# multiplefish/VPLines-SLAM

Hardware: AMD Instinct MI355X
Metric: sliding-window BA solves/sec (10 KF, 200 pts + 80 lines, 5 iters) (higher is better)
Workload: dtype f64

## Files before the change

vplines-slam_amd/csrc/ba_stage.h:

```cpp
#pragma once
#include <hip/hip_runtime.h>

#include <algorithm>
#include <cstring>
#include <memory>
#include <vector>

struct CopySeg {
  const char* src;
  char* dst;
  unsigned bytes;
  unsigned u0;
};
static_assert(sizeof(CopySeg) == 24, "CopySeg layout");

__global__ __launch_bounds__(256) void k_copy_segments(const CopySeg* tab, int nseg, unsigned total_units) {
  for (unsigned u = blockIdx.x * 256u + threadIdx.x; u < total_units; u += gridDim.x * 256u) {
    int lo = 0, hi = nseg - 1;
    while (lo < hi) {
      const int mid = (lo + hi + 1) >> 1;
      if (tab[mid].u0 <= u) lo = mid; else hi = mid - 1;
    }
    const CopySeg sg = tab[lo];
    const unsigned off = (u - sg.u0) * 16u;
    const unsigned rem = sg.bytes - off;
    const char* src = sg.src + off;
    char* dst = sg.dst + off;
    if (rem >= 16u && (((uintptr_t)src | (uintptr_t)dst) & 15u) == 0) {
      *reinterpret_cast<uint4*>(dst) = *reinterpret_cast<const uint4*>(src);
    } else {
      const unsigned nb = rem < 16u ? rem : 16u;
      for (unsigned b = 0; b < nb; b += 4) *reinterpret_cast<uint32_t*>(dst + b) = *reinterpret_cast<const uint32_t*>(src + b);
    }
  }
}

template <typename T>
struct Span {
  T* p = nullptr;
  size_t n = 0;
  T& operator[](size_t i) const { return p[i]; }
  T* data() const { return p; }
  size_t size() const { return n; }
  bool empty() const { return n == 0; }
  T* begin() const { return p; }
  T* end() const { return p + n; }
};

struct Stage {
  char* h = nullptr;
  char* d = nullptr;
  size_t cap = 0, used = 0;
  std::vector<CopySeg> segs;
  unsigned units = 0;
  bool overflow = false;
  bool dry = false;
  std::vector<std::unique_ptr<char[]>> spill;

  hipError_t reserve(size_t need) {
    used = 0; segs.clear(); units = 0; overflow = false; spill.clear();
    if (need <= cap) return hipSuccess;
    release();
    const size_t want = need + need / 4 + (1u << 16);
    hipError_t e = hipHostMalloc((void**)&h, want, hipHostMallocDefault);
    if (e != hipSuccess) return e;
    e = hipMalloc((void**)&d, want);
    if (e != hipSuccess) return e;
    cap = want;
    return hipSuccess;
  }
  void release() {
    if (h) (void)hipHostFree(h);
    if (d) (void)hipFree(d);
    h = d = nullptr; cap = 0;
  }
  size_t bound() const { return ((used + 63) & ~(size_t)63) + segs.size() * sizeof(CopySeg); }
  template <typename T>
  Span<T> take(size_t n) {
    used = (used + 63) & ~(size_t)63;
    Span<T> sp;
    sp.n = n;
    if (!dry && used + n * sizeof(T) <= cap) sp.p = reinterpret_cast<T*>(h + used);
    else if (!dry) { overflow = true; spill.emplace_back(new char[n * sizeof(T) + 1]); sp.p = reinterpret_cast<T*>(spill.back().get()); }
    used += n * sizeof(T);
    return sp;
  }
  template <typename T>
// ... 52 lines not shown
```

vplines-slam_amd/csrc/ba_step.h:

```cpp
#pragma once
#include "ba_common.h"
#include "ba_solve.h"

namespace vpl {

constexpr int SCHUR_THREADS = 256;
constexpr int CHOL_THREADS = 256;
constexpr int BACK_THREADS = 256;

__device__ __forceinline__ void lds_ticket_wait(int* t, int seq) {
  while (__hip_atomic_load(t, __ATOMIC_RELAXED, __HIP_MEMORY_SCOPE_WORKGROUP) != seq) __builtin_amdgcn_s_sleep(1);
  __builtin_amdgcn_fence(__ATOMIC_ACQUIRE, "workgroup", "local");
}
__device__ __forceinline__ void lds_ticket_pass(int* t, int seq, int lane) {
  __builtin_amdgcn_fence(__ATOMIC_RELEASE, "workgroup", "local");
  if (lane == 0) __hip_atomic_store(t, seq + 1, __ATOMIC_RELAXED, __HIP_MEMORY_SCOPE_WORKGROUP);
}

__device__ __forceinline__ int compact2vis(int c, int s, int WS) {
  if (c < WS - 6) { const int v = 6 * s + c; return v < 66 ? v : -1; }
  if (c < WS) return 66 + (c - (WS - 6));
  return c < WS + 2 ? 72 + (c - WS) : -1;
}

// ... 542 lines not shown
__global__ __launch_bounds__(SCHUR_THREADS, 2) void k_schur_mixed(DevBatch B) {
  extern __shared__ double sm[];
  if (blockIdx.x == 0 && threadIdx.x == 0) { B.ord_cnt[2 * ((B.ord_it + 1) & 1)] = 0; B.ord_cnt[2 * ((B.ord_it + 1) & 1) + 1] = 0; }
  schur_body<3, true>(B, ordered_window(B), sm);
}
inline size_t schur_smem(int maxP, int maxL, int ntc = 5) {
  const int r1 = std::max(4 * maxP + 28 * maxL, (int)CSQ_N);
  const int maxKS = maxP / 4 + maxL + NF + 2;
  return (size_t)(r1 + 3 * maxP + 22 * maxL + 176 + 24) * sizeof(double) + (size_t)(8 + 4 * maxKS + ntc * (ntc + 1) / 2 * 256) * sizeof(int);
}

constexpr int DN = 90;
constexpr int DNT = 6;
constexpr int DNAP = DNT * (DNT + 1) / 2 * 256;
constexpr int XLD = 80;
constexpr int CHOL_MIN_WAVES = 2;
constexpr int XROWS_A = 36, XROWS_B = 48;
__device__ __forceinline__ constexpr int xcol(int ch, int J) { return ch == 0 ? 16 * (J > 3 ? J - 1 : J) : 16 * (J - 1); }
__device__ __forceinline__ constexpr int tile_row(int t) { return t < 1 ? 0 : t < 3 ? 1 : t < 6 ? 2 : t < 10 ? 3 : t < 15 ? 4 : 5; }

__device__ __forceinline__ int chain_frame(int ch, int b) { return ch == 0 ? 1 + b : 10 - b; }
__device__ __forceinline__ int chain_col(int ch, int b, int lane) {
  if (lane < 18) {
    const int ds = (b & 1) ? 9 : 0;
    const int f = chain_frame(ch, b);
    const int fr = (lane >= ds && lane < ds + 9) ? f : (ch == 0 ? f + 1 : f - 1);
    return 15 * fr + 6 + (lane < 9 ? lane : lane - 9);
  }
  if (ch == 0) {
    if (lane < 27) return 6 + (lane - 18);
    if (lane < 63) return 15 * ((lane - 27) / 6) + (lane - 27) % 6;
    return NC;
  }
  if (lane < 54) return 15 * (5 + (lane - 18) / 6) + (lane - 18) % 6;
  return lane == 54 ? NC : -1;
}
__device__ __forceinline__ int cam2dense(int c) {
  if (c < 0) return -1;
  if (c == NC) return DN;
  const int v = cam2vis(c);
  if (v >= 0) return v;
  if (c < 15) return 72 + (c - 6);
  return (c >= 81 && c < 90) ? c : -1;
}
__device__ __forceinline__ int dense2cam(int d) { return d < NV ? vis2cam(d) : (d < 81 ? 6 + (d - 72) : d); }
__device__ __forceinline__ int chain_dense(int ch, int lane) {
  if (lane < 18) {
    const bool s5 = ch == 0 ? lane < 9 : lane >= 9;
    return s5 ? 81 + (lane < 9 ? lane : lane - 9) : -1;
  }
  return cam2dense(chain_col(ch, 0, lane));
}

__device__ __forceinline__ void chol_body(const DevBatch& B, const int w, double* sm) {
  const int tid = threadIdx.x, T = CHOL_THREADS;
  const int lane = tid & 63, wv = ((tid >> 6) + ((blockIdx.x >> 8) & 1) * 2) & 3;
  TrState* tr = &B.tr[w];
  if (tr->status != 0 || tr->reuse != 0 || B.path[w] != 0) return;
  count_active(B, 1);
  constexpr int REG = (XROWS_A + XROWS_B) * XLD > DNAP ? (XROWS_A + XROWS_B) * XLD : DNAP;
  double* XA = sm;
  double* XBm = sm + XROWS_A * XLD;
  double* S = sm;
  double* scv = sm + REG;
  double* dgv = scv + 176;
  double* ycam = dgv + 176;
  double* yv = ycam + 176;
  double* isd = yv + 96;
  double* Linv = isd + 96;
  double* red = Linv + 256;
  int* flag = (int*)(red + 24);
  double* rsL = (double*)(flag + 8);

  const size_t fb = (size_t)w * B.nfull;
  const double* gscale = B.scale + fb;
  const double* gdiag = B.diag + fb;
  const double* ggrad = B.grad + fb;
  double* ggn = B.gn + fb;
  const double* Hcc = B.Hcc + (size_t)w * NCP;
  const double* gc = B.gc + (size_t)w * NC;
  const double* sacc = B.sacc + (size_t)w * SACC_N;
  const double mu = tr->mu;
  for (int c = tid; c < 176; c += T) { scv[c] = c < NC ? gscale[c] : 0.0; dgv[c] = c < NC ? gdiag[c] : 1.0; ycam[c] = 0.0; }
  if (tid < 4) flag[tid] = 0;
  for (int i = tid; i < (XROWS_A + XROWS_B) * XLD; i += T) sm[i] = 0.0;
  __syncthreads();
  VPL_STAMP(B, w, 8);

  double U[45];
#pragma unroll
  for (int i = 0; i < 45; ++i) U[i] = 0.0;
#define Xs(b, k) U[9 * (b) + (k)]
  if (wv < 2) {
    const int ch = wv, nblk = ch == 0 ? 4 : 5;
    double* Xout = ch == 0 ? XA : XBm;
    const int xd = chain_dense(ch, lane);
    const int xp = xd < 0 ? -1 : xcol(ch, xd >> 4) + (xd & 15);
    bool bad = false;
    auto load_strip = [&](int b, double (&raw)[9]) {
      const int col = chain_col(ch, b, lane);
      const int f = chain_frame(ch, b);
#pragma unroll
      for (int i = 0; i < 9; ++i) {
        const int r = 15 * f + 6 + i;
        raw[i] = 0.0;
        if (col == NC) raw[i] = gc[r];
        else if (col >= 0) raw[i] = Hcc[col > r ? tri(col, r) : tri(r, col)];
      }
    };
    double rawn[9];
    load_strip(0, rawn);
#pragma unroll
    for (int b = 0; b < 5; ++b) {
      if (b < nblk) {
        const int ds = (b & 1) ? 9 : 0, ns = 9 - ds;
        const int col = chain_col(ch, b, lane);
        const int f = chain_frame(ch, b);
        double R[9];
        {
          const double scol = col == NC ? 1.0 : (col >= 0 ? scv[col] : 0.0);
#pragma unroll
          for (int i = 0; i < 9; ++i) {
            const int r = 15 * f + 6 + i;
            R[i] = rawn[i] * (scv[r] * scol);
            if (col == r) R[i] += mu * dgv[r] * dgv[r];
          }
        }
        if (b + 1 < nblk) load_strip(b + 1, rawn);
        if (b > 0) {
          const bool fresh = lane >= ns && lane < ns + 9;
#pragma unroll
          for (int k = 0; k < 9; ++k) {
            const double xk = fresh ? 0.0 : Xs(b - 1, k);
#pragma unroll
            for (int i = 0; i < 9; ++i) R[i] -= readlane_f64(Xs(b - 1, k), ds + i) * xk;
          }
        }
// ... 77 lines not shown
#pragma unroll 1
    for (int ks = 0; ks < XROWS_B / 4; ++ks) {
      const int need = min(5, (4 * ks + 3) / 9 + 1);
      while (have < need) {
        have = __hip_atomic_load(&flag[2], __ATOMIC_RELAXED, __HIP_MEMORY_SCOPE_WORKGROUP);
        if (have >= need) __builtin_amdgcn_fence(__ATOMIC_ACQUIRE, "workgroup");
      }
      const double* row = XBm + (4 * ks + kk) * XLD + m;
      double x[6];
#pragma unroll
      for (int J = 0; J < 6; ++J) x[J] = J == 0 ? 0.0 : row[xcol(1, J)];
#pragma unroll
      for (int t = 0; t < 21; ++t) {
        const int I = tile_row(t), J = t - I * (I + 1) / 2;
        if ((t & 1) != p || J == 0) continue;
        acc[t >> 1] = __builtin_amdgcn_mfma_f64_16x16x4f64(x[I], x[J], acc[t >> 1], 0, 0, 0);
      }
    }
#pragma unroll
    for (int i = 0; i < 11; ++i) {
      const v4d h = hs[i] - acc[i];
      U[4 * i] = h.x; U[4 * i + 1] = h.y; U[4 * i + 2] = h.z; U[4 * i + 3] = h.w;
    }
  }
  __syncthreads();
  VPL_STAMP(B, w, 9);

  if (wv >= 2) {
    const int p = __builtin_amdgcn_readfirstlane(wv - 2);
    const int m = lane & 15, kk = lane >> 4;
#pragma unroll
    for (int t = 0; t < 21; ++t) {
      if ((t & 1) != p) continue;
      double* St = S + (t << 8);
#pragma unroll
      for (int v = 0; v < 4; ++v) {
        const int r = kk + 4 * v;
        St[tsw(r, m)] = (t == 20 && r == DN - 80 && m == DN - 80) ? 1.0 : U[4 * (t >> 1) + v];
      }
    }
  }
  __syncthreads();
  VPL_STAMP(B, w, 10);

  if (!tile_cholesky(S, Linv, isd, flag, DNT, DN, CHOL_THREADS / 64, lane, wv, nullptr)) {
    if (tid == 0) B.path[w] = 2;
    return;
  }
  VPL_STAMP(B, w, 11);
  tile_back_substitute(S, isd, yv, DNT, DN, tid, T, lane, wv);
  for (int d = tid; d < DN; d += T) ycam[dense2cam(d)] = yv[d];
  __syncthreads();
  VPL_STAMP(B, w, 12);
  if (wv < 2) {
    const int ch = wv, nblk = ch == 0 ? 4 : 5;
#pragma unroll
    for (int b = 4; b >= 0; --b) {
      if (b < nblk) {
        const int ds = (b & 1) ? 9 : 0;
        const int col = chain_col(ch, b, lane);
        const int f = chain_frame(ch, b);
        const bool pivl = lane >= ds && lane < ds + 9;
        const double cf = col == NC ? 1.0 : ((col < 0 || pivl) ? 0.0 : -ycam[col]);
        double t[9];
#pragma unroll
        for (int k = 0; k < 9; ++k) t[k] = wave_sum_dpp(Xs(b, k) * cf);
#pragma unroll
        for (int j = 8; j >= 0; --j) {
          const double yj = t[j] * rsL[(5 * ch + b) * 9 + j];
#pragma unroll
          for (int k = 0; k < j; ++k) t[k] -= readlane_f64(Xs(b, k), ds + j) * yj;
          t[j] = yj;
        }
        if (lane == 0) {
#pragma unroll
          for (int j = 0; j < 9; ++j) ycam[15 * f + 6 + j] = t[j];
        }
        __builtin_amdgcn_fence(__ATOMIC_RELEASE, "workgroup");
        __builtin_amdgcn_wave_barrier();
        __builtin_amdgcn_fence(__ATOMIC_ACQUIRE, "workgroup");
      }
    }
  }
  __syncthreads();
  double a2 = 0.0, a3 = 0.0;
  double* ycs = B.ycs + (size_t)w * 176;
  for (int c = tid; c < 176; c += T) {
    double u = 0.0;
    if (c < NC) {
      const double y = ycam[c];
      u = scv[c] * y;
      const double gnv = -dgv[c] * y;
      ggn[c] = gnv;
      a2 += gnv * gnv;
      a3 += ggrad[c] * gnv;
    }
    ycs[c] = u;
  }
  a2 = block_sum(a2, red);
  a3 = block_sum(a3, red);
  if (tid == 0) { B.sx[(size_t)w * 8] = a2; B.sx[(size_t)w * 8 + 1] = a3; }
  VPL_STAMP(B, w, 13);
}
#undef Xs
__global__ __launch_bounds__(CHOL_THREADS, CHOL_MIN_WAVES) void k_chol(DevBatch B) {
  extern __shared__ double sm[];
  chol_body(B, ordered_window(B), sm);
}
constexpr size_t CHOL_SMEM = (size_t)(((XROWS_A + XROWS_B) * XLD > DNAP ? (XROWS_A + XROWS_B) * XLD : DNAP) + 3 * 176 + 2 * 96 + 256 + 24 + 96) * sizeof(double) + (8 + 128) * sizeof(int);

template <bool FUSED = false>
__device__ __forceinline__ void back_body(const DevBatch& B, const int w, double* sm) {
  const int tid = threadIdx.x, T = BACK_THREADS;
  const int lane = tid & 63;
  TrState* tr = &B.tr[w];
  if (tr->status != 0) return;
  const int path = B.path[w];
  if (path != 0) {
    if (FUSED) return;
    __syncthreads();
    if (tid == 0 && path == 2) B.path[w] = 0;
    return;
  }
  const int nP = B.nP[w], nL = B.nL[w];
  const int WS = B.WS;
  double* uc = sm;
  double* lrhs = uc + 176;
  double* lgn = lrhs + 4 * B.maxL;
  double* gdelta = lgn + B.nfull;
  double* red = gdelta + B.nfull;
  int* pSt = (int*)(red + 24);
  int* lSt = pSt + B.maxP;
  const size_t fb = (size_t)w * B.nfull;
  const double* gscale = B.scale + fb;
  const double* gdiag = B.diag + fb;
  const double* ggrad = B.grad + fb;
  double* ggn = B.gn + fb;
  const double* lch = B.lchol + (size_t)w * B.maxL * 10;
  const int LP = NC, LL = NC + B.maxP;
  const bool reuse0 = tr->reuse != 0;
  count_active(B, reuse0 ? 2 : 1);
  VPL_STAMP(B, w, 5);
  if (!reuse0) {
    const double mu = tr->mu;
    for (int p = tid; p < nP; p += T) pSt[p] = B.pt_start[(size_t)w * B.maxP + p];
    for (int l = tid; l < nL; l += T) lSt[l] = B.ln_start[(size_t)w * B.maxL + l];
    for (int c = tid; c < 176; c += T) uc[c] = c < NV ? B.ycs[(size_t)w * 176 + vis2cam(c)] : 0.0;
    for (int c = tid; c < NC; c += T) lgn[c] = ggn[c];
    __syncthreads();
    double a2 = 0.0, a3 = 0.0;
    {
      const int sub = lane & 7, grp = tid >> 3;
      const int nblk = WS / 6;
      constexpr int NPH = 4;
      for (int p0 = 0; p0 < nP; p0 += NPH * (T / 8)) {
        double wyv[NPH], sv[NPH], dv[NPH], hv[NPH], gv2[NPH], grv[NPH];
        size_t piv[NPH];
#pragma unroll
        for (int h = 0; h < NPH; ++h) {
          const int p = p0 + h * (T / 8) + grp;
          piv[h] = (size_t)w * B.maxP + (p < nP ? p : 0);
          wyv[h] = 0.0; sv[h] = dv[h] = 1.0; hv[h] = gv2[h] = grv[h] = 0.0;
          if (p < nP) {
            const int s0 = pSt[p];
            for (int blk = sub; blk < nblk; blk += 8) {
              const bool exb = blk == nblk - 1;
              const int vb = exb ? 66 : 6 * (s0 + blk);
              if (!exb && vb >= 66) continue;
              const double* Wr = B.Wp + piv[h] * WS + 6 * blk;
#pragma unroll
              for (int k = 0; k < 6; ++k) wyv[h] += Wr[k] * uc[vb + k];
            }
            if (sub == 0) {
              sv[h] = gscale[LP + p]; dv[h] = gdiag[LP + p]; hv[h] = B.Hpp[piv[h]]; gv2[h] = B.gp[piv[h]];
              grv[h] = ggrad[LP + p];
            }
          }
        }
#pragma unroll
        for (int h = 0; h < NPH; ++h) {
          const int p = p0 + h * (T / 8) + grp;
          double wy = wyv[h];
          wy += __shfl_xor(wy, 1, 64); wy += __shfl_xor(wy, 2, 64); wy += __shfl_xor(wy, 4, 64);
          if (p < nP && sub == 0) {
            const double s = sv[h], d = dv[h];
            const double Al = s * s * hv[h] + mu * d * d;
            const double y = s * (gv2[h] - wy) / Al;
            const double gnv = -d * y;
            ggn[LP + p] = gnv; lgn[LP + p] = gnv;
            a2 += gnv * gnv;
            a3 += grv[h] * gnv;
          }
        }
      }
      constexpr int NLH = 5;
      for (int r0 = 0; r0 < 4 * nL; r0 += NLH * (T / 8)) {
        double wyv[NLH], glv[NLH];
#pragma unroll
        for (int h = 0; h < NLH; ++h) {
          const int r = r0 + h * (T / 8) + grp, l = r >> 2, a = r & 3;
          wyv[h] = 0.0; glv[h] = 0.0;
          if (l < nL) {
            const size_t li = (size_t)w * B.maxL + l;
            const int s0 = lSt[l];
            for (int blk = sub; blk < nblk; blk += 8) {
              const bool exb = blk == nblk - 1;
              const int vb = exb ? 66 : 6 * (s0 + blk);
              if (!exb && vb >= 66) continue;
              const double* Wr = B.Wl + (li * 4 + a) * WS + 6 * blk;
#pragma unroll
              for (int k = 0; k < 6; ++k) wyv[h] += Wr[k] * uc[vb + k];
            }
            if (sub == 0) glv[h] = B.gl[li * 4 + a];
          }
        }
#pragma unroll
        for (int h = 0; h < NLH; ++h) {
          const int r = r0 + h * (T / 8) + grp;
          double wy = wyv[h];
          wy += __shfl_xor(wy, 1, 64); wy += __shfl_xor(wy, 2, 64); wy += __shfl_xor(wy, 4, 64);
          if (r < 4 * nL && sub == 0) lrhs[r] = gscale[LL + r] * (glv[h] - wy);
        }
      }
      __syncthreads();
      for (int l = tid; l < nL; l += T) {
        double C[10], t4[4], gd4[4], gr4[4];
#pragma unroll
        for (int k = 0; k < 10; ++k) C[k] = lch[l * 10 + k];
#pragma unroll
        for (int k = 0; k < 4; ++k) { gd4[k] = gdiag[LL + 4 * l + k]; gr4[k] = ggrad[LL + 4 * l + k]; }
#pragma unroll
        for (int k = 0; k < 4; ++k) t4[k] = lrhs[4 * l + k];
#pragma unroll
        for (int k = 0; k < 4; ++k) {
          double s2 = t4[k];
#pragma unroll
          for (int j = 0; j < 4; ++j) if (j < k) s2 -= C[tri(k, j)] * t4[j];
          t4[k] = s2 / C[tri(k, k)];
        }
#pragma unroll
        for (int k = 3; k >= 0; --k) {
          double s2 = t4[k];
#pragma unroll
          for (int j = 0; j < 4; ++j) if (j > k) s2 -= C[tri(j, k)] * t4[j];
          t4[k] = s2 / C[tri(k, k)];
        }
#pragma unroll
        for (int k = 0; k < 4; ++k) {
          const double gnv = -gd4[k] * t4[k];
          ggn[LL + 4 * l + k] = gnv; lgn[LL + 4 * l + k] = gnv;
          a2 += gnv * gnv;
          a3 += gr4[k] * gnv;
        }
      }
    }
    a2 = block_sum(a2, red);
    a3 = block_sum(a3, red);
    if (tid == 0) {
      tr->a2 = a2 + B.sx[(size_t)w * 8];
      tr->a3 = a3 + B.sx[(size_t)w * 8 + 1];
      tr->reuse = 1;
    }
    __syncthreads();
  }
  VPL_STAMP(B, w, 6);
  const double radius = tr->radius, alpha = tr->alpha, a1 = tr->a1, a2 = tr->a2, a3 = tr->a3, mu = tr->mu;
  const double gradient_norm = sqrt(a1), gauss_newton_norm = sqrt(a2);
  double c1, c2, dnorm;
  if (gauss_newton_norm <= radius) {
    c1 = 0.0; c2 = 1.0; dnorm = gauss_newton_norm;
  } else if (gradient_norm * alpha >= radius) {
    c1 = radius / gradient_norm; c2 = 0.0; dnorm = radius;
  } else {
    const double b_dot_a = -alpha * a3;
    const double a_sq = (alpha * gradient_norm) * (alpha * gradient_norm);
    const double bma = a_sq - 2 * b_dot_a + a2;
    const double c = b_dot_a - a_sq;
    const double d = sqrt(c * c + bma * (radius * radius - a_sq));
    const double beta = (c <= 0) ? (d - c) / bma : (radius * radius - a_sq) / (d + c);
    c1 = alpha * (1.0 - beta); c2 = beta;
    dnorm = sqrt(c1 * c1 * a1 - 2.0 * c1 * c2 * a3 + c2 * c2 * a2);
  }
  const double q_cauchy = a1 / alpha;
  const double sg = -c1 * a1 + c2 * a3;
  const double vHy = a1 + mu * a3;
  const double yHy = -a3 - mu * a2;
  const double sHs = c1 * c1 * q_cauchy + 2.0 * c1 * c2 * vHy + c2 * c2 * yHy;
  const double model_cost_change = -(sg + 0.5 * sHs);
  const bool valid = model_cost_change > 0.0;
  if (!valid) {
    if (tid == 0) {
      tr->step_valid = 0;
      tr->iter += 1;
      tr->num_invalid += 1;
      if (tr->num_invalid >= kMaxInvalid) { tr->status = 2; tr->iter -= 1; }
      else if (tr->iter >= B.opt.num_iterations) tr->status = 3;
      tr->mu *= kMuIncrease;
      tr->reuse = 0;
    }
    return;
  }
  const int nfull_used = NC + B.maxP + 4 * nL;
  for (int k = tid; k < nfull_used; k += T) {
    const bool live = k < NC || (k >= LP && k < LP + nP) || k >= LL;
    if (live) gdelta[k] = gscale[k] * (-c1 * ggrad[k] + c2 * (reuse0 ? ggn[k] : lgn[k])) / gdiag[k];
// ... 23 lines not shown
    }
  }
  for (int p = tid; p < nP; p += T) {
    const size_t pi = (size_t)w * B.maxP + p;
    const double d = gdelta[LP + p];
    B.invd_c[pi] = B.invd[pi] + d;
    sn += d * d; xn += B.invd[pi] * B.invd[pi];
  }
  for (int l = tid; l < nL; l += T) {
    const size_t li = (size_t)w * B.maxL + l;
    double out[4];
    line_orth_plus(B.orth + li * 4, gdelta + LL + 4 * l, out);
    for (int k = 0; k < 4; ++k) {
      const double x = B.orth[li * 4 + k];
      B.orth_c[li * 4 + k] = out[k];
      sn += (x - out[k]) * (x - out[k]); xn += x * x;
    }
    const Plk Lc_ = orth_to_plk(out);
    double* lwc = B.lw_c + li * 6;
    lwc[0] = Lc_.n.x; lwc[1] = Lc_.n.y; lwc[2] = Lc_.n.z; lwc[3] = Lc_.v.x; lwc[4] = Lc_.v.y; lwc[5] = Lc_.v.z;
  }
  sn = block_sum(sn, red);
  xn = block_sum(xn, red);
  VPL_STAMP(B, w, 7);
  if (tid == 0) {
    tr->dogleg_step_norm = dnorm;
    tr->model_cost_change = model_cost_change;
    tr->step_norm = sqrt(sn);
    tr->x_norm = sqrt(xn);
    tr->step_valid = 1;
    tr->num_invalid = 0;
  }
}
#ifndef VPL_BACK_WAVES
#define VPL_BACK_WAVES 2
#endif
__global__ __launch_bounds__(BACK_THREADS, VPL_BACK_WAVES) void k_back(DevBatch B) {
  extern __shared__ double sm[];
  back_body(B, ordered_window(B), sm);
}
inline size_t back_smem(int maxP, int maxL) {
  const int nfull = NC + maxP + 4 * maxL;
  return (size_t)(176 + 4 * maxL + 2 * nfull + 24) * sizeof(double) + (size_t)(maxP + maxL) * sizeof(int);
}

static_assert(SCHUR_THREADS == CHOL_THREADS && CHOL_THREADS == BACK_THREADS, "k_step runs the three bodies with one work-group shape");
template <int NTC, bool MIXED>
__global__ __launch_bounds__(SCHUR_THREADS, 2) void k_step(DevBatch B) {
  extern __shared__ double sm[];
  if (blockIdx.x == 0 && threadIdx.x == 0) { B.ord_cnt[2 * ((B.ord_it + 1) & 1)] = 0; B.ord_cnt[2 * ((B.ord_it + 1) & 1) + 1] = 0; }
  const int w = ordered_window(B);
  schur_body<NTC, MIXED>(B, w, sm);
  __syncthreads();
  chol_body(B, w, sm);
  __syncthreads();
  back_body<true>(B, w, sm);
}
inline size_t step_smem(int maxP, int maxL, int ntc = 5) {
  return std::max(std::max(schur_smem(maxP, maxL, ntc), (size_t)CHOL_SMEM), back_smem(maxP, maxL));
}

}
```

vplines-slam_amd/csrc/ba_upload.h:

```cpp
#pragma once
#include "ba_ctx.h"
#include "ba_odo.h"
#include "ba_pack.h"
#include "host_common.h"

static void to_dev_preint(const vpl_preintegration& p, DevPreint& d) {
  d.sum_dt = p.sum_dt;
  for (int k = 0; k < 3; ++k) { d.dp[k] = p.delta_p[k]; d.dv[k] = p.delta_v[k]; d.lba[k] = p.linearized_ba[k]; d.lbg[k] = p.linearized_bg[k]; }
  for (int k = 0; k < 4; ++k) d.dq[k] = p.delta_q[k];
  auto blk = [&](double* o, int r0, int c0) {
    for (int i = 0; i < 3; ++i)
      for (int j = 0; j < 3; ++j) o[3 * i + j] = p.jacobian[(r0 + i) * 15 + c0 + j];
  };
  blk(d.dp_dba, 0, 9); blk(d.dp_dbg, 0, 12); blk(d.dq_dbg, 3, 12); blk(d.dv_dba, 6, 9); blk(d.dv_dbg, 6, 12);
  std::memcpy(d.cov, p.covariance, sizeof(d.cov));
  std::memset(d.sqrt_info, 0, sizeof(d.sqrt_info));
}

struct UploadArena {
  Span<double> pose, sb, ex, invd, plk, pt_obs, ln_obs, fail_ref, orth, pr_x0, pr_r0;
  Span<int> nP, nL, pt_start, pt_nobs, pt_off, ln_start, ln_nobs, ln_off, ln_tri, pu_cnt, pu_cnt0, sk_tab, sk_wave, path, nLO, lo_ln,
      ll_tab, ll_np, ps_list, ps_cnt, orth_in, pr_n, pr_nb, pr_kind, pr_frame, pr_idx, mg_n, mg_nb, mg_kind, mg_frame, mg_idx, mg_cam, mg_m;
  Span<DevPreint> pre;
  std::vector<Span<double>> J0;
// ... 450 lines not shown
  HIPCHK(c, SG.reserve(upload_bound(B, W, win, same_layout, dev_prior, odo)));
  UploadArena A;
  take_upload(SG, A, B, W, win, dev_prior, odo);
  std::unique_ptr<int[]> lane(new int[W * B.maxPR * 1024]), sub(new int[W * B.maxPR * 512]);
  long schur_wide_w = 0, schur_total_w = 0;
  for (size_t w = 0; w < W; ++w) {
    const HostTab* T = dev_prior ? &ctab[w] : nullptr;
    if ((rc = pack_tracks(c, A, w, win[w], all_lines))) return rc;
    if (odo) pack_gather(c, A, w, win[w], *odo);
    else pack_values(c, A, w, win[w]);
    if (!same_layout &&
        (rc = build_layout(c, A, w, win[w], &lane[w * B.maxPR * 1024], &sub[w * B.maxPR * 512], &schur_wide_w, &schur_total_w)))
      return rc;
    if ((rc = pack_prior(c, A, w, win[w], T))) return rc;
    if ((rc = keep_blocks(c, A, w, win[w], T))) return rc;
  }
  if ((rc = choose_marg(c, A.mg_n, W))) return rc;
  if (!same_layout) pack_units(SG, A, W, B.maxPR, lane.get(), sub.get());
  std::memcpy(A.mg_m.p, c->h_mg_m.data(), W * 4);
  c->h_mg_n.assign(A.mg_n.begin(), A.mg_n.end());
  c->h_mg_nb.assign(A.mg_nb.begin(), A.mg_nb.end());
  if (odo)
    for (size_t w = 0; w < W; ++w)
      A.odo_marg[w] = (opt->marginalization_flag != VPL_MARGIN_NONE && c->h_passthrough[w] < 0) ? 1 + A.mg_nb[w] : 0;
  if (!same_layout) c->schur_mostly_wide = schur_total_w > 0 && 20 * schur_wide_w > 7 * schur_total_w;
  if (c->force_general) std::fill(A.path.begin(), A.path.end(), 1);
  if (SG.overflow) return fail(c, VPL_E_CAPACITY, "internal: staging arena bound too small");
  stage_upload(SG, A, B, W, same_layout, dev_prior, odo);
  if (chained && (rc = hand_over_priors(c, ctab, prev_prS))) return rc;
  HIPCHK(c, stage_run(c->stage, c->stream, true, &c->last_upload_bytes));
  if (odo) {
    hipLaunchKernelGGL(k_odo_gather, dim3(nW), dim3(ODO_THREADS), 0, c->stream, B, odo->store, (const int*)odo->d_psrc, (const int*)odo->d_lsrc);
    if (odo->tab) hipLaunchKernelGGL(k_odo_prior_load, dim3(nW), dim3(ODO_THREADS), 0, c->stream, B, odo->prior, (const int*)odo->d_has);
    HIPCHK(c, hipGetLastError());
  }
  if (c->leg_timing) HIPCHK(c, hipEventRecord(c->leg_ev[1], c->stream));
  HIPCHK(c, hipStreamSynchronize(c->stream));
  c->layout_valid = true;
  return VPL_OK;
}
static int upload_impl(vpl_ctx* c, int nW, const vpl_window* win, const vpl_ba_options* opt, bool all_lines, bool chained = false,
                       const OdoSrc* odo = nullptr) {
  const int rc = upload_body(c, nW, win, opt, all_lines, chained, odo);
  if (c) {
    if (rc != VPL_OK && c->upload_open) { c->nW = 0; c->prior_resident = false; }
    c->upload_open = false;
  }
  return rc;
}

static int restore_states(vpl_ctx* c, bool plk) {
  const DevBatch& B = c->B;
  const size_t W = c->nW;
  HIPCHK(c, hipMemcpyAsync(B.pose, B.pose_0, W * 77 * 8, hipMemcpyDeviceToDevice, c->stream));
  HIPCHK(c, hipMemcpyAsync(B.sb, B.sb_0, W * 99 * 8, hipMemcpyDeviceToDevice, c->stream));
  HIPCHK(c, hipMemcpyAsync(B.ex, B.ex_0, W * 7 * 8, hipMemcpyDeviceToDevice, c->stream));
  HIPCHK(c, hipMemcpyAsync(B.invd, B.invd_0, W * B.maxP * 8, hipMemcpyDeviceToDevice, c->stream));
  if (plk) HIPCHK(c, hipMemcpyAsync(B.plk, B.plk_0, W * B.maxL * 6 * 8, hipMemcpyDeviceToDevice, c->stream));
  return VPL_OK;
}
```

vplines-slam_amd/csrc/vplines_ba.hip:

```cpp
#include <hip/hip_runtime.h>

#include <algorithm>
#include <chrono>
#include <memory>
#include <cstdlib>
#include <cstring>
#include <string>
#include <vector>

#include "vplines_ba.h"
#include "ba_types.h"
#include "ba_lin.h"
#include "ba_pack.h"
#include "ba_solve.h"
#include "ba_step.h"
#include "ba_marg.h"
#include "ba_prior_eig.h"
#include "ba_lineopt.h"
#include "ba_factors.h"
#include "ba_odo.h"
#include "odo_tracks.h"
#include "host_common.h"

using namespace vpl;
// ... 95 lines not shown
  AL(pose_c, W * 77); AL(sb_c, W * 99); AL(ex_c, W * 7); AL(invd_c, W * B.maxP); AL(orth_c, W * B.maxL * 4); AL(lw, W * B.maxL * 6); AL(lw_c, W * B.maxL * 6);
  AL(lin_part, W * LIN_PART); AL(lin_pcost, W); AL(lin_flag, W);
  AL(pose_0, W * 77); AL(sb_0, W * 99); AL(ex_0, W * 7); AL(invd_0, W * B.maxP); AL(plk_0, W * B.maxL * 6);
  AL(plk, W * B.maxL * 6); AL(gauge, W * 4); AL(fail_ref, W * 13); AL(orth_in, W);
  AL(nP, W); AL(nL, W);
  AL(pt_start, W * B.maxP); AL(pt_nobs, W * B.maxP); AL(pt_off, W * B.maxP); AL(pt_obs, W * B.maxPO * 3);
  AL(ps_list, W * B.maxP); AL(ps_cnt, W * (NF + 1)); AL(pu_lane, W * B.maxPR * 1024); AL(pu_sub, W * B.maxPR * 512); AL(pu_cnt, W); AL(pu_cnt0, W);
  AL(ln_start, W * B.maxL); AL(ln_nobs, W * B.maxL); AL(ln_off, W * B.maxL); AL(ln_obs, W * B.maxLO * 8);
  AL(nLO, W); AL(lo_ln, W * B.maxLO);
  AL(ll_tab, W * B.llSlots * 2); AL(ll_np, W);
  AL(pre, W * NF);
  AL(pr_n, W); AL(pr_nb, W); AL(pr_kind, W * MAXPB); AL(pr_frame, W * MAXPB); AL(pr_idx, W * MAXPB);
  AL(pr_x0, W * MAXPB * 9); AL(pr_J0, W * MAXPN * MAXPN); AL(pr_r0, W * MAXPN); AL(pr_H, W * MAXPN * MAXPN); AL(pr_g0, W * MAXPN);
  AL(pr_map, W * MAXPN);
  AL(Hcc, W * NCP); AL(gc, W * NC); AL(asm_tab, 2 * NCP); AL(Hpp, W * B.maxP); AL(gp, W * B.maxP); AL(Wp, W * B.maxP * NV);
  AL(Hll, W * B.maxL * 16); AL(gl, W * B.maxL * 4); AL(Wl, W * B.maxL * 4 * NV); AL(lchol, W * B.maxL * 10);
  AL(tr, W);
  AL(scale, W * B.nfull); AL(diag, W * B.nfull); AL(grad, W * B.nfull); AL(gn, W * B.nfull);
  AL(mg_n, W); AL(mg_nb, W); AL(mg_kind, W * MAXPB); AL(mg_frame, W * MAXPB); AL(mg_idx, W * MAXPB);
  AL(mg_cam, W * MAXPB); AL(mg_x0, W * MAXPB * 9); AL(mg_J0, W * MAXKEEP * MAXKEEP); AL(mg_r0, W * MAXKEEP);
  AL(mg_A, W * MAXKEEP * MAXKEEP); AL(mg_b, W * MAXKEEP); AL(mg_m, W); AL(dbg, W * 64); AL(ln_removed, W * B.maxL); AL(ln_tri, W * B.maxL);
  if (e == hipSuccess) e = dalloc(c, &c->d_act, (size_t)ACT_SLOTS * 4);
  AL(order, 2 * W); AL(ord_cnt, 4);
  AL(sk_tab, W * B.maxKS * 4); AL(sk_wave, W * 8 * SK_WSTRIDE); AL(sacc, W * SACC_N); AL(nz_tab, NZ_N); AL(ycs, W * 176); AL(sx, W * 8); AL(path, W);
#undef AL
  if (e != hipSuccess) return VPL_E_HIP;
  if (lin_smem_base(c->maxP, c->maxL) > LIN_LDS_BUDGET) return VPL_E_CAPACITY;
  B.prhN = lin_prh_n(c->maxP, c->maxL);
  {
    std::vector<int> tab(2 * NCP);
    for (int r = 0, e2 = 0; r < NC; ++r)
      for (int cc = 0; cc <= r; ++cc, ++e2) lin_asm_entry(r, cc, &tab[2 * e2]);
    if (hipMemcpy(B.asm_tab, tab.data(), tab.size() * sizeof(int), hipMemcpyHostToDevice) != hipSuccess) return VPL_E_HIP;
  }
  {
    std::vector<int> nz;
    for (int r = 0; r < NC; ++r)
      for (int cc = 0; cc <= r; ++cc) {
        const bool vis = cam2vis(r) >= 0 && cam2vis(cc) >= 0;
        const int fr = r < 165 ? r / 15 : -1, fc = cc < 165 ? cc / 15 : -1;
        const bool band = fr >= 0 && fc >= 0 && (fr == fc || fr == fc + 1);
        const bool sb0 = cc >= 6 && cc < 15 && cam2vis(r) >= 0;
        if (vis || band || sb0) nz.push_back(tri(r, cc) | r << 14 | cc << 22);
      }
    if ((int)nz.size() != NZ_N || hipMemcpy(B.nz_tab, nz.data(), nz.size() * sizeof(int), hipMemcpyHostToDevice) != hipSuccess) return VPL_E_HIP;
  }
  static size_t lin_max = 0, solve_max = 0, schur_max = 0, back_max = 0, step_max = 0;
  lin_max = std::max(lin_max, lin_smem(c->maxP, c->maxL));
  solve_max = std::max(solve_max, solve_smem(c->maxP, c->maxL));
  schur_max = std::max(schur_max, schur_smem(c->maxP, c->maxL));
  back_max = std::max(back_max, back_smem(c->maxP, c->maxL));
  step_max = std::max(step_max, step_smem(c->maxP, c->maxL));
  if (schur_max > 159 * 1024 || back_max > 159 * 1024) return VPL_E_CAPACITY;
  const std::pair<const void*, size_t> lds[] = {
      {(const void*)k_lin2, lin_max}, {(const void*)k_lin<1>, lin_max}, {(const void*)k_lin<2>, lin_max},
      {(const void*)k_solve, solve_max}, {(const void*)k_schur<3>, schur_max}, {(const void*)k_schur<5>, schur_max},
      {(const void*)k_schur_mixed, schur_max}, {(const void*)k_chol, CHOL_SMEM}, {(const void*)k_back, back_max},
      {(const void*)k_step<3, false>, step_max}, {(const void*)k_step<3, true>, step_max}, {(const void*)k_step<5, false>, step_max},
      {(const void*)k_prep, PREP_SMEM}, {(const void*)k_marg<MARG_THREADS>, 159 * 1024}, {(const void*)k_marg<256>, MARG_LDS_SMALL},
      {(const void*)k_prior_eigen, prior_eig_layout(MAXKEEP).bytes}, {(const void*)k_init_align, init_lds_bytes(INIT_NMAX)}};
  for (const auto& k : lds)
    if (hipFuncSetAttribute(k.first, hipFuncAttributeMaxDynamicSharedMemorySize, (int)k.second) != hipSuccess) return VPL_E_HIP;
  vpl_ba_default_options(&c->opt);
  if (const char* gv = std::getenv("VPL_BA_GRAPH")) c->use_graph = std::atoi(gv) != 0;
  if (const char* gv = std::getenv("VPL_BA_GENERAL")) c->force_general = std::atoi(gv) != 0;
  if (const char* gv = std::getenv("VPL_BA_STEP_FUSED")) c->step_fused = std::atoi(gv) != 0;
  if (const char* gv = std::getenv("VPL_BA_SCHUR_WIDE")) { c->schur_wide_all = std::atoi(gv) > 0; c->schur_never_wide = std::atoi(gv) < 0; }
  return VPL_OK;
}

int vpl_ctx_create(vpl_ctx** out, int device, int max_windows, int max_points, int max_point_obs, int max_lines,
                   int max_line_obs) {
  if (!out || max_windows < 1 || max_points < 0 || max_lines < 0) return VPL_E_INVALID;
  int ndev = 0;
  if (hipGetDeviceCount(&ndev) != hipSuccess || ndev == 0 || device >= ndev) return VPL_E_NODEVICE;
  if (hipSetDevice(device) != hipSuccess) return VPL_E_NODEVICE;
  vpl_ctx* c = new vpl_ctx();
  const int rc = ctx_init(c, device, max_windows, max_points, max_point_obs, max_lines, max_line_obs);
  if (rc != VPL_OK) {
    free_arrays(c);
    delete c;
    return rc;
  }
  *out = c;
  return VPL_OK;
}

void vpl_ctx_destroy(vpl_ctx* c) {
  if (!c) return;
  (void)hipSetDevice(c->device);
  (void)hipDeviceSynchronize();
  drop_graph(c);
  free_arrays(c);
  c->stage.release();
  for (hipEvent_t& e : c->leg_ev) if (e) (void)hipEventDestroy(e);
  delete c;
}

int vpl_ctx_set_stream(vpl_ctx* c, void* s) {
  if (!c) return VPL_E_INVALID;
  const int rs = settle(c);
  if (rs) return rs;
  if (c->stream != (hipStream_t)s) {
    HIPCHK(c, hipSetDevice(c->device));
    (void)hipStreamSynchronize(c->stream);
    (void)hipGetLastError();
// ... 847 lines not shown
```

Measured before the change: 263,700.

## Overlap back-substitution rows with Cholesky chains and batch state-restore copies

In the fused step kernel, the two idle wavefronts that previously waited during the camera triangular-solve chains now compute the point and line back-substitution rows. They coordinate through a workgroup atomic pair-sync, so back_body only has to accumulate the reductions. Separately, the five device-to-device restore memcpys are replaced by a single copy kernel that takes its segment table by value. This adds LDS-layout coupling and a new capacity check that can reject large maxP/maxL configurations. It also risks correctness issues in the custom inter-wave sync.

```diff
diff --git a/vplines-slam_amd/csrc/ba_stage.h b/vplines-slam_amd/csrc/ba_stage.h
--- a/vplines-slam_amd/csrc/ba_stage.h
+++ b/vplines-slam_amd/csrc/ba_stage.h
@@ -14,6 +14,19 @@
 };
 static_assert(sizeof(CopySeg) == 24, "CopySeg layout");
 
+__device__ __forceinline__ void copy_unit(const CopySeg& sg, unsigned u) {
+  const unsigned off = (u - sg.u0) * 16u;
+  const unsigned rem = sg.bytes - off;
+  const char* src = sg.src + off;
+  char* dst = sg.dst + off;
+  if (rem >= 16u && (((uintptr_t)src | (uintptr_t)dst) & 15u) == 0) {
+    *reinterpret_cast<uint4*>(dst) = *reinterpret_cast<const uint4*>(src);
+  } else {
+    const unsigned nb = rem < 16u ? rem : 16u;
+    for (unsigned b = 0; b < nb; b += 4) *reinterpret_cast<uint32_t*>(dst + b) = *reinterpret_cast<const uint32_t*>(src + b);
+  }
+}
+
 __global__ __launch_bounds__(256) void k_copy_segments(const CopySeg* tab, int nseg, unsigned total_units) {
   for (unsigned u = blockIdx.x * 256u + threadIdx.x; u < total_units; u += gridDim.x * 256u) {
     int lo = 0, hi = nseg - 1;
@@ -21,18 +34,36 @@
       const int mid = (lo + hi + 1) >> 1;
       if (tab[mid].u0 <= u) lo = mid; else hi = mid - 1;
     }
-    const CopySeg sg = tab[lo];
-    const unsigned off = (u - sg.u0) * 16u;
-    const unsigned rem = sg.bytes - off;
-    const char* src = sg.src + off;
-    char* dst = sg.dst + off;
-    if (rem >= 16u && (((uintptr_t)src | (uintptr_t)dst) & 15u) == 0) {
-      *reinterpret_cast<uint4*>(dst) = *reinterpret_cast<const uint4*>(src);
-    } else {
-      const unsigned nb = rem < 16u ? rem : 16u;
-      for (unsigned b = 0; b < nb; b += 4) *reinterpret_cast<uint32_t*>(dst + b) = *reinterpret_cast<const uint32_t*>(src + b);
-    }
+    copy_unit(tab[lo], u);
   }
+}
+
+constexpr int COPY_FEW_MAX = 5;
+struct CopyFew {
+  CopySeg seg[COPY_FEW_MAX];
+  unsigned total_units;
+  void add(int k, const void* src, void* dst, size_t bytes) {
+    seg[k] = CopySeg{reinterpret_cast<const char*>(src), reinterpret_cast<char*>(dst), (unsigned)bytes, total_units};
+    total_units += (unsigned)((bytes + 15) / 16);
+  }
+  void close(int n) {
+    for (int k = n; k < COPY_FEW_MAX; ++k) seg[k] = CopySeg{nullptr, nullptr, 0u, total_units};
+  }
+};
+__global__ __launch_bounds__(256) void k_copy_few(const CopyFew A) {
+  for (unsigned u = blockIdx.x * 256u + threadIdx.x; u < A.total_units; u += gridDim.x * 256u) {
+    CopySeg sg = A.seg[0];
+#pragma unroll
+    for (int k = 1; k < COPY_FEW_MAX; ++k)
+      if (A.seg[k].u0 <= u) sg = A.seg[k];
+    copy_unit(sg, u);
+  }
+}
+static hipError_t copy_few(const CopyFew& F, hipStream_t stream) {
+  if (!F.total_units) return hipSuccess;
+  const unsigned blocks = std::min<unsigned>((F.total_units + 255) / 256, 2048u);
+  hipLaunchKernelGGL(k_copy_few, dim3(blocks), dim3(256), 0, stream, F);
+  return hipGetLastError();
 }
 
 template <typename T>
diff --git a/vplines-slam_amd/csrc/ba_step.h b/vplines-slam_amd/csrc/ba_step.h
--- a/vplines-slam_amd/csrc/ba_step.h
+++ b/vplines-slam_amd/csrc/ba_step.h
@@ -618,13 +618,158 @@
   return cam2dense(chain_col(ch, 0, lane));
 }
 
+constexpr int CHOL_REG = (XROWS_A + XROWS_B) * XLD > DNAP ? (XROWS_A + XROWS_B) * XLD : DNAP;
+struct BackLds {
+  double *uc, *lrhs, *lgn, *gdelta, *red;
+  int *pSt, *lSt;
+};
+template <bool EARLY>
+__device__ __forceinline__ BackLds back_lds(const DevBatch& B, double* sm) {
+  BackLds L;
+  L.uc = sm;
+  L.lrhs = L.uc + 176;
+  L.lgn = L.lrhs + 4 * B.maxL;
+  if (EARLY) {
+    L.pSt = (int*)(L.lgn + B.nfull);
+    L.lSt = L.pSt + B.maxP;
+    L.gdelta = (double*)(((uintptr_t)(L.lSt + B.maxL) + 7) & ~(uintptr_t)7);
+    L.red = L.gdelta + B.nfull;
+  } else {
+    L.gdelta = L.lgn + B.nfull;
+    L.red = L.gdelta + B.nfull;
+    L.pSt = (int*)(L.red + 24);
+    L.lSt = L.pSt + B.maxP;
+  }
+  return L;
+}
+inline size_t back_rows_bytes(int maxP, int maxL) {
+  return (size_t)(176 + 4 * maxL + NC + maxP + 4 * maxL) * sizeof(double) + (size_t)(maxP + maxL) * sizeof(int);
+}
+template <int TT, bool SUM, typename Sync>
+__device__ __forceinline__ void back_rows(const DevBatch& B, const int w, const BackLds& L, const int t, const double mu, double& a2,
+                                          double& a3, Sync sync) {
+  const int nP = B.nP[w], nL = B.nL[w];
+  const int WS = B.WS;
+  const size_t fb = (size_t)w * B.nfull;
+  const double* gscale = B.scale + fb;
+  const double* gdiag = B.diag + fb;
+  const double* ggrad = B.grad + fb;
+  double* ggn = B.gn + fb;
+  const double* lch = B.lchol + (size_t)w * B.maxL * 10;
+  const int LP = NC, LL = NC + B.maxP;
+  const int sub = t & 7, grp = t >> 3;
+  const int nblk = WS / 6;
+  constexpr int NPH = 4;
+  for (int p0 = 0; p0 < nP; p0 += NPH * (TT / 8)) {
+    double wyv[NPH], sv[NPH], dv[NPH], hv[NPH], gv2[NPH], grv[NPH];
+    size_t piv[NPH];
+#pragma unroll
+    for (int h = 0; h < NPH; ++h) {
+      const int p = p0 + h * (TT / 8) + grp;
+      piv[h] = (size_t)w * B.maxP + (p < nP ? p : 0);
+      wyv[h] = 0.0; sv[h] = dv[h] = 1.0; hv[h] = gv2[h] = grv[h] = 0.0;
+      if (p < nP) {
+        const int s0 = L.pSt[p];
+        for (int blk = sub; blk < nblk; blk += 8) {
+          const bool exb = blk == nblk - 1;
+          const int vb = exb ? 66 : 6 * (s0 + blk);
+          if (!exb && vb >= 66) continue;
+          const double* Wr = B.Wp + piv[h] * WS + 6 * blk;
+#pragma unroll
+          for (int k = 0; k < 6; ++k) wyv[h] += Wr[k] * L.uc[vb + k];
+        }
+        if (sub == 0) {
+          sv[h] = gscale[LP + p]; dv[h] = gdiag[LP + p]; hv[h] = B.Hpp[piv[h]]; gv2[h] = B.gp[piv[h]];
+          grv[h] = ggrad[LP + p];
+        }
+      }
+    }
+#pragma unroll
+    for (int h = 0; h < NPH; ++h) {
+      const int p = p0 + h * (TT / 8) + grp;
+      double wy = wyv[h];
+      wy += __shfl_xor(wy, 1, 64); wy += __shfl_xor(wy, 2, 64); wy += __shfl_xor(wy, 4, 64);
+      if (p < nP && sub == 0) {
+        const double s = sv[h], d = dv[h];
+        const double Al = s * s * hv[h] + mu * d * d;
+        const double y = s * (gv2[h] - wy) / Al;
+        const double gnv = -d * y;
+        ggn[LP + p] = gnv; L.lgn[LP + p] = gnv;
+        if (SUM) a2 += gnv * gnv;
+        if (SUM) a3 += grv[h] * gnv;
+      }
+    }
+  }
+  constexpr int NLH = 5;
+  for (int r0 = 0; r0 < 4 * nL; r0 += NLH * (TT / 8)) {
+    double wyv[NLH], glv[NLH];
+#pragma unroll
+    for (int h = 0; h < NLH; ++h) {
+      const int r = r0 + h * (TT / 8) + grp, l = r >> 2, a = r & 3;
+      wyv[h] = 0.0; glv[h] = 0.0;
+      if (l < nL) {
+        const size_t li = (size_t)w * B.maxL + l;
+        const int s0 = L.lSt[l];
+        for (int blk = sub; blk < nblk; blk += 8) {
+          const bool exb = blk == nblk - 1;
+          const int vb = exb ? 66 : 6 * (s0 + blk);
+          if (!exb && vb >= 66) continue;
+          const double* Wr = B.Wl + (li * 4 + a) * WS + 6 * blk;
+#pragma unroll
+          for (int k = 0; k < 6; ++k) wyv[h] += Wr[k] * L.uc[vb + k];
+        }
+        if (sub == 0) glv[h] = B.gl[li * 4 + a];
+      }
+    }
+#pragma unroll
+    for (int h = 0; h < NLH; ++h) {
+      const int r = r0 + h * (TT / 8) + grp;
+      double wy = wyv[h];
+      wy += __shfl_xor(wy, 1, 64); wy += __shfl_xor(wy, 2, 64); wy += __shfl_xor(wy, 4, 64);
+      if (r < 4 * nL && sub == 0) L.lrhs[r] = gscale[LL + r] * (glv[h] - wy);
+    }
+  }
+  sync();
+  for (int l = t; l < nL; l += TT) {
+    double C[10], t4[4], gd4[4], gr4[4];
+#pragma unroll
+    for (int k = 0; k < 10; ++k) C[k] = lch[l * 10 + k];
+#pragma unroll
+    for (int k = 0; k < 4; ++k) { gd4[k] = gdiag[LL + 4 * l + k]; gr4[k] = ggrad[LL + 4 * l + k]; }
+#pragma unroll
+    for (int k = 0; k < 4; ++k) t4[k] = L.lrhs[4 * l + k];
+#pragma unroll
+    for (int k = 0; k < 4; ++k) {
+      double s2 = t4[k];
+#pragma unroll
+      for (int j = 0; j < 4; ++j) if (j < k) s2 -= C[tri(k, j)] * t4[j];
+      t4[k] = s2 / C[tri(k, k)];
+    }
+#pragma unroll
+    for (int k = 3; k >= 0; --k) {
+      double s2 = t4[k];
+#pragma unroll
+      for (int j = 0; j < 4; ++j) if (j > k) s2 -= C[tri(j, k)] * t4[j];
+      t4[k] = s2 / C[tri(k, k)];
+    }
+#pragma unroll
+    for (int k = 0; k < 4; ++k) {
+      const double gnv = -gd4[k] * t4[k];
+      ggn[LL + 4 * l + k] = gnv; L.lgn[LL + 4 * l + k] = gnv;
+      if (SUM) a2 += gnv * gnv;
+      if (SUM) a3 += gr4[k] * gnv;
+    }
+  }
+}
+
+template <bool ROWS = false>
 __device__ __forceinline__ void chol_body(const DevBatch& B, const int w, double* sm) {
   const int tid = threadIdx.x, T = CHOL_THREADS;
   const int lane = tid & 63, wv = ((tid >> 6) + ((blockIdx.x >> 8) & 1) * 2) & 3;
   TrState* tr = &B.tr[w];
   if (tr->status != 0 || tr->reuse != 0 || B.path[w] != 0) return;
   count_active(B, 1);
-  constexpr int REG = (XROWS_A + XROWS_B) * XLD > DNAP ? (XROWS_A + XROWS_B) * XLD : DNAP;
+  constexpr int REG = CHOL_REG;
   double* XA = sm;
   double* XBm = sm + XROWS_A * XLD;
   double* S = sm;
@@ -648,7 +793,7 @@
   const double* sacc = B.sacc + (size_t)w * SACC_N;
   const double mu = tr->mu;
   for (int c = tid; c < 176; c += T) { scv[c] = c < NC ? gscale[c] : 0.0; dgv[c] = c < NC ? gdiag[c] : 1.0; ycam[c] = 0.0; }
-  if (tid < 4) flag[tid] = 0;
+  if (tid < (ROWS ? 8 : 4)) flag[tid] = 0;
   for (int i = tid; i < (XROWS_A + XROWS_B) * XLD; i += T) sm[i] = 0.0;
   __syncthreads();
   VPL_STAMP(B, w, 8);
@@ -832,7 +977,7 @@
   for (int d = tid; d < DN; d += T) ycam[dense2cam(d)] = yv[d];
   __syncthreads();
   VPL_STAMP(B, w, 12);
-  if (wv < 2) {
+  if (ROWS ? __builtin_amdgcn_readfirstlane(wv) < 2 : wv < 2) {
     const int ch = wv, nblk = ch == 0 ? 4 : 5;
 #pragma unroll
     for (int b = 4; b >= 0; --b) {
@@ -861,6 +1006,29 @@
         __builtin_amdgcn_fence(__ATOMIC_ACQUIRE, "workgroup");
       }
     }
+  } else if (ROWS) {
+    const int t = (wv - 2) * 64 + lane;
+    const BackLds L = back_lds<true>(B, sm);
+#ifdef VPL_STAMPS
+    if (t == 0) B.dbg[(size_t)w * 64 + 14] = (long long)__builtin_readcyclecounter();
+#endif
+    for (int p = t; p < B.nP[w]; p += 128) L.pSt[p] = B.pt_start[(size_t)w * B.maxP + p];
+    for (int l = t; l < B.nL[w]; l += 128) L.lSt[l] = B.ln_start[(size_t)w * B.maxL + l];
+    for (int c = t; c < 176; c += 128) L.uc[c] = c < NV ? scv[vis2cam(c)] * ycam[vis2cam(c)] : 0.0;
+    int arrived = 0;
+    auto pair_sync = [&]() {
+      arrived += 2;
+      __builtin_amdgcn_fence(__ATOMIC_RELEASE, "workgroup");
+      if (lane == 0) __hip_atomic_fetch_add(&flag[4], 1, __ATOMIC_RELAXED, __HIP_MEMORY_SCOPE_WORKGROUP);
+      while (__hip_atomic_load(&flag[4], __ATOMIC_RELAXED, __HIP_MEMORY_SCOPE_WORKGROUP) < arrived) __builtin_amdgcn_s_sleep(1);
+      __builtin_amdgcn_fence(__ATOMIC_ACQUIRE, "workgroup");
+    };
+    pair_sync();
+    double a2u = 0.0, a3u = 0.0;
+    back_rows<128, false>(B, w, L, t, mu, a2u, a3u, pair_sync);
+#ifdef VPL_STAMPS
+    if (t == 0) B.dbg[(size_t)w * 64 + 15] = (long long)__builtin_readcyclecounter();
+#endif
   }
   __syncthreads();
   double a2 = 0.0, a3 = 0.0;
@@ -887,10 +1055,11 @@
   extern __shared__ double sm[];
   chol_body(B, ordered_window(B), sm);
 }
-constexpr size_t CHOL_SMEM = (size_t)(((XROWS_A + XROWS_B) * XLD > DNAP ? (XROWS_A + XROWS_B) * XLD : DNAP) + 3 * 176 + 2 * 96 + 256 + 24 + 96) * sizeof(double) + (8 + 128) * sizeof(int);
-
-template <bool FUSED = false>
+constexpr size_t CHOL_SMEM = (size_t)(CHOL_REG + 3 * 176 + 2 * 96 + 256 + 24 + 96) * sizeof(double) + (8 + 128) * sizeof(int);
+
+template <bool FUSED = false, bool ROWS_DONE = false>
 __device__ __forceinline__ void back_body(const DevBatch& B, const int w, double* sm) {
+  static_assert(FUSED || !ROWS_DONE, "the rows move into chol_body in the one-launch form only");
   const int tid = threadIdx.x, T = BACK_THREADS;
   const int lane = tid & 63;
   TrState* tr = &B.tr[w];
@@ -904,13 +1073,9 @@
   }
   const int nP = B.nP[w], nL = B.nL[w];
   const int WS = B.WS;
-  double* uc = sm;
-  double* lrhs = uc + 176;
-  double* lgn = lrhs + 4 * B.maxL;
-  double* gdelta = lgn + B.nfull;
-  double* red = gdelta + B.nfull;
-  int* pSt = (int*)(red + 24);
-  int* lSt = pSt + B.maxP;
+  const BackLds L = back_lds<ROWS_DONE>(B, sm);
+  double *uc = L.uc, *lgn = L.lgn, *gdelta = L.gdelta, *red = L.red;
+  int *pSt = L.pSt, *lSt = L.lSt;
   const size_t fb = (size_t)w * B.nfull;
   const double* gscale = B.scale + fb;
   const double* gdiag = B.diag + fb;
@@ -923,114 +1088,36 @@
   VPL_STAMP(B, w, 5);
   if (!reuse0) {
     const double mu = tr->mu;
-    for (int p = tid; p < nP; p += T) pSt[p] = B.pt_start[(size_t)w * B.maxP + p];
-    for (int l = tid; l < nL; l += T) lSt[l] = B.ln_start[(size_t)w * B.maxL + l];
-    for (int c = tid; c < 176; c += T) uc[c] = c < NV ? B.ycs[(size_t)w * 176 + vis2cam(c)] : 0.0;
+    if (!ROWS_DONE) {
+      for (int p = tid; p < nP; p += T) pSt[p] = B.pt_start[(size_t)w * B.maxP + p];
+      for (int l = tid; l < nL; l += T) lSt[l] = B.ln_start[(size_t)w * B.maxL + l];
+      for (int c = tid; c < 176; c += T) uc[c] = c < NV ? B.ycs[(size_t)w * 176 + vis2cam(c)] : 0.0;
+    }
     for (int c = tid; c < NC; c += T) lgn[c] = ggn[c];
     __syncthreads();
     double a2 = 0.0, a3 = 0.0;
-    {
+    if (!ROWS_DONE) {
+      back_rows<BACK_THREADS, true>(B, w, L, tid, mu, a2, a3, [] { __syncthreads(); });
+    } else {
       const int sub = lane & 7, grp = tid >> 3;
-      const int nblk = WS / 6;
       constexpr int NPH = 4;
       for (int p0 = 0; p0 < nP; p0 += NPH * (T / 8)) {
-        double wyv[NPH], sv[NPH], dv[NPH], hv[NPH], gv2[NPH], grv[NPH];
-        size_t piv[NPH];
 #pragma unroll
         for (int h = 0; h < NPH; ++h) {
           const int p = p0 + h * (T / 8) + grp;
-          piv[h] = (size_t)w * B.maxP + (p < nP ? p : 0);
-          wyv[h] = 0.0; sv[h] = dv[h] = 1.0; hv[h] = gv2[h] = grv[h] = 0.0;
-          if (p < nP) {
-            const int s0 = pSt[p];
-            for (int blk = sub; blk < nblk; blk += 8) {
-              const bool exb = blk == nblk - 1;
-              const int vb = exb ? 66 : 6 * (s0 + blk);
-              if (!exb && vb >= 66) continue;
-              const double* Wr = B.Wp + piv[h] * WS + 6 * blk;
-#pragma unroll
-              for (int k = 0; k < 6; ++k) wyv[h] += Wr[k] * uc[vb + k];
-            }
-            if (sub == 0) {
-              sv[h] = gscale[LP + p]; dv[h] = gdiag[LP + p]; hv[h] = B.Hpp[piv[h]]; gv2[h] = B.gp[piv[h]];
-              grv[h] = ggrad[LP + p];
-            }
+          if (p < nP && sub == 0) {
+            const double gnv = lgn[LP + p];
+            a2 += gnv * gnv;
+            a3 += ggrad[LP + p] * gnv;
           }
         }
-#pragma unroll
-        for (int h = 0; h < NPH; ++h) {
-          const int p = p0 + h * (T / 8) + grp;
-          double wy = wyv[h];
-          wy += __shfl_xor(wy, 1, 64); wy += __shfl_xor(wy, 2, 64); wy += __shfl_xor(wy, 4, 64);
-          if (p < nP && sub == 0) {
-            const double s = sv[h], d = dv[h];
-            const double Al = s * s * hv[h] + mu * d * d;
-            const double y = s * (gv2[h] - wy) / Al;
-            const double gnv = -d * y;
-            ggn[LP + p] = gnv; lgn[LP + p] = gnv;
-            a2 += gnv * gnv;
-            a3 += grv[h] * gnv;
-          }
-        }
-      }
-      constexpr int NLH = 5;
-      for (int r0 = 0; r0 < 4 * nL; r0 += NLH * (T / 8)) {
-        double wyv[NLH], glv[NLH];
-#pragma unroll
-        for (int h = 0; h < NLH; ++h) {
-          const int r = r0 + h * (T / 8) + grp, l = r >> 2, a = r & 3;
-          wyv[h] = 0.0; glv[h] = 0.0;
-          if (l < nL) {
-            const size_t li = (size_t)w * B.maxL + l;
-            const int s0 = lSt[l];
-            for (int blk = sub; blk < nblk; blk += 8) {
-              const bool exb = blk == nblk - 1;
-              const int vb = exb ? 66 : 6 * (s0 + blk);
-              if (!exb && vb >= 66) continue;
-              const double* Wr = B.Wl + (li * 4 + a) * WS + 6 * blk;
-#pragma unroll
-              for (int k = 0; k < 6; ++k) wyv[h] += Wr[k] * uc[vb + k];
-            }
-            if (sub == 0) glv[h] = B.gl[li * 4 + a];
-          }
-        }
-#pragma unroll
-        for (int h = 0; h < NLH; ++h) {
-          const int r = r0 + h * (T / 8) + grp;
-          double wy = wyv[h];
-          wy += __shfl_xor(wy, 1, 64); wy += __shfl_xor(wy, 2, 64); wy += __shfl_xor(wy, 4, 64);
-          if (r < 4 * nL && sub == 0) lrhs[r] = gscale[LL + r] * (glv[h] - wy);
-        }
-      }
-      __syncthreads();
+      }
       for (int l = tid; l < nL; l += T) {
-        double C[10], t4[4], gd4[4], gr4[4];
-#pragma unroll
-        for (int k = 0; k < 10; ++k) C[k] = lch[l * 10 + k];
-#pragma unroll
-        for (int k = 0; k < 4; ++k) { gd4[k] = gdiag[LL + 4 * l + k]; gr4[k] = ggrad[LL + 4 * l + k]; }
-#pragma unroll
-        for (int k = 0; k < 4; ++k) t4[k] = lrhs[4 * l + k];
 #pragma unroll
         for (int k = 0; k < 4; ++k) {
-          double s2 = t4[k];
-#pragma unroll
-          for (int j = 0; j < 4; ++j) if (j < k) s2 -= C[tri(k, j)] * t4[j];
-          t4[k] = s2 / C[tri(k, k)];
-        }
-#pragma unroll
-        for (int k = 3; k >= 0; --k) {
-          double s2 = t4[k];
-#pragma unroll
-          for (int j = 0; j < 4; ++j) if (j > k) s2 -= C[tri(j, k)] * t4[j];
-          t4[k] = s2 / C[tri(k, k)];
-        }
-#pragma unroll
-        for (int k = 0; k < 4; ++k) {
-          const double gnv = -gd4[k] * t4[k];
-          ggn[LL + 4 * l + k] = gnv; lgn[LL + 4 * l + k] = gnv;
+          const double gnv = lgn[LL + 4 * l + k];
           a2 += gnv * gnv;
-          a3 += gr4[k] * gnv;
+          a3 += ggrad[LL + 4 * l + k] * gnv;
         }
       }
     }
@@ -1160,12 +1247,12 @@
   const int w = ordered_window(B);
   schur_body<NTC, MIXED>(B, w, sm);
   __syncthreads();
-  chol_body(B, w, sm);
+  chol_body<true>(B, w, sm);
   __syncthreads();
-  back_body<true>(B, w, sm);
+  back_body<true, true>(B, w, sm);
 }
 inline size_t step_smem(int maxP, int maxL, int ntc = 5) {
-  return std::max(std::max(schur_smem(maxP, maxL, ntc), (size_t)CHOL_SMEM), back_smem(maxP, maxL));
-}
-
-}
+  return std::max(std::max(schur_smem(maxP, maxL, ntc), (size_t)CHOL_SMEM), back_smem(maxP, maxL) + 8);
+}
+
+}
diff --git a/vplines-slam_amd/csrc/ba_upload.h b/vplines-slam_amd/csrc/ba_upload.h
--- a/vplines-slam_amd/csrc/ba_upload.h
+++ b/vplines-slam_amd/csrc/ba_upload.h
@@ -526,10 +526,14 @@
 static int restore_states(vpl_ctx* c, bool plk) {
   const DevBatch& B = c->B;
   const size_t W = c->nW;
-  HIPCHK(c, hipMemcpyAsync(B.pose, B.pose_0, W * 77 * 8, hipMemcpyDeviceToDevice, c->stream));
-  HIPCHK(c, hipMemcpyAsync(B.sb, B.sb_0, W * 99 * 8, hipMemcpyDeviceToDevice, c->stream));
-  HIPCHK(c, hipMemcpyAsync(B.ex, B.ex_0, W * 7 * 8, hipMemcpyDeviceToDevice, c->stream));
-  HIPCHK(c, hipMemcpyAsync(B.invd, B.invd_0, W * B.maxP * 8, hipMemcpyDeviceToDevice, c->stream));
-  if (plk) HIPCHK(c, hipMemcpyAsync(B.plk, B.plk_0, W * B.maxL * 6 * 8, hipMemcpyDeviceToDevice, c->stream));
-  return VPL_OK;
-}
+  CopyFew F{};
+  int n = 0;
+  F.add(n++, B.pose_0, B.pose, W * 77 * 8);
+  F.add(n++, B.sb_0, B.sb, W * 99 * 8);
+  F.add(n++, B.ex_0, B.ex, W * 7 * 8);
+  F.add(n++, B.invd_0, B.invd, W * B.maxP * 8);
+  if (plk) F.add(n++, B.plk_0, B.plk, W * B.maxL * 6 * 8);
+  F.close(n);
+  HIPCHK(c, copy_few(F, c->stream));
+  return VPL_OK;
+}
diff --git a/vplines-slam_amd/csrc/vplines_ba.hip b/vplines-slam_amd/csrc/vplines_ba.hip
--- a/vplines-slam_amd/csrc/vplines_ba.hip
+++ b/vplines-slam_amd/csrc/vplines_ba.hip
@@ -171,6 +171,7 @@
   back_max = std::max(back_max, back_smem(c->maxP, c->maxL));
   step_max = std::max(step_max, step_smem(c->maxP, c->maxL));
   if (schur_max > 159 * 1024 || back_max > 159 * 1024) return VPL_E_CAPACITY;
+  if (back_rows_bytes(c->maxP, c->maxL) > CHOL_REG * sizeof(double)) return VPL_E_CAPACITY;
   const std::pair<const void*, size_t> lds[] = {
       {(const void*)k_lin2, lin_max}, {(const void*)k_lin<1>, lin_max}, {(const void*)k_lin<2>, lin_max},
       {(const void*)k_solve, solve_max}, {(const void*)k_schur<3>, schur_max}, {(const void*)k_schur<5>, schur_max},
```

Result: slower. 258,300 (-2.0%).
